# PRBonn/OverlapNet

Measured on AMD Instinct MI355X. Metric: scan-pairs/s (64x900 range images), higher is better.
Workload: dtype f32 (scaled 3-term fp16 split on the fp16 MFMA: 22 significand bits per operand, fp32 accumulate)

## Files before the change

overlapnet_amd/csrc/c3_dense.hip:

```cpp
#include "ovn_internal.h"

typedef _Float16 f16x8 __attribute__((ext_vector_type(8)));
typedef _Float16 f16x4 __attribute__((ext_vector_type(4)));

namespace {

struct ArithF16 {
  typedef _Float16 elem;
  typedef f16x8 v8;
  typedef f16x4 v4;
  static __device__ __forceinline__ f32x4 mfma(v8 a, v8 b, f32x4 c) { return __builtin_amdgcn_mfma_f32_16x16x32_f16(a, b, c, 0, 0, 0); }
};

constexpr int G = OVN_G;
constexpr int OW = OVN_O3_HW;
constexpr int CI = OVN_C2_OUT;
constexpr int CO = OVN_C3_OUT;
constexpr int NBAND = 3;
constexpr int MAX_ROWS = 8;
constexpr int MAX_MT = (MAX_ROWS * OW + 15) / 16;
constexpr int IN_PIX_MAX = (MAX_ROWS + 2) * G;
constexpr int PLANE = IN_PIX_MAX * 8 + 8;
constexpr int NPL = CI / 8;
constexpr size_t LDS_BYTES = 2 * (size_t)NPL * PLANE * sizeof(_Float16) + 64;
// ... 1 lines not shown

__device__ __forceinline__ int band_start(int b) { return b == 0 ? 0 : (b == 1 ? 8 : 15); }
__device__ __forceinline__ int band_rows(int b) { return b == 0 ? 8 : 7; }

constexpr int MT_SPLIT = 6;
template <class A, int NWV, int MSPLIT>
__global__ __launch_bounds__(64 * NWV) void c3_dense_kernel(const float* __restrict__ o2, const typename A::elem* __restrict__ wp,
                                                           const float* __restrict__ b3, const float* __restrict__ wd,
                                                           const unsigned* __restrict__ o2max, float sw3,
                                                           float* __restrict__ partial, float* __restrict__ o3,
                                                           unsigned* __restrict__ arrived, const float* __restrict__ bd,
                                                           float* __restrict__ overlap, float* __restrict__ logit) {
  typedef typename A::elem elem_t;
  typedef typename A::v8 v8_t;
  typedef typename A::v4 v4_t;
  extern __shared__ __attribute__((aligned(16))) unsigned char smem[];
  elem_t* ih = reinterpret_cast<elem_t*>(smem);
  elem_t* il = ih + NPL * PLANE;
  float* red = reinterpret_cast<float*>(il + NPL * PLANE);

  constexpr int HALVES = NW / NWV;
  constexpr int MTW = MSPLIT == 1 ? MAX_MT : MT_SPLIT;
  const int sub = blockIdx.x % (HALVES * MSPLIT);
  const int unit = blockIdx.x / (HALVES * MSPLIT), half = sub % HALVES, mh = sub / HALVES;
  const int mt0 = MT_SPLIT * mh;
  const int pair = unit / NBAND;
  const int band = unit - pair * NBAND;
  const int r0 = band_start(band);
  const int nrows = band_rows(band);
  const int npix = nrows * OW;
  const int nmt = (npix + 15) >> 4;
// ... 37 lines not shown
        const int c = 4 * (i - pix * (CI / 4));
        v4_t h, l;
#pragma unroll
        for (int e = 0; e < 4; ++e) {
          const float x = v[k][e] * s2;
          h[e] = (elem_t)x;
          l[e] = (elem_t)(x - (float)h[e]);
        }
        const int o = (c >> 3) * PLANE + pix * 8 + (c & 7);
        *reinterpret_cast<v4_t*>(ih + o) = h;
        *reinterpret_cast<v4_t*>(il + o) = l;
      }
    }
  }

  int abase[MTW];
#pragma unroll
  for (int mt = 0; mt < MTW; ++mt) {
    int p = 16 * (mt0 + mt) + lrow;
    if (p >= npix) p = npix - 1;
    const int oy = p / OW;
    const int ox = p - oy * OW;
    abase[mt] = g * PLANE + (oy * G + ox) * 8;
  }

  f32x4 acc[MTW][2];
#pragma unroll
  for (int mt = 0; mt < MTW; ++mt) {
    acc[mt][0] = (f32x4){0.f, 0.f, 0.f, 0.f};
    acc[mt][1] = (f32x4){0.f, 0.f, 0.f, 0.f};
  }

#define C3_MFMA2(M0, M1, A0H, A0L, A1H, A1L, SRC)                                                  \
  acc[M0][0] = A::mfma(A0H, SRC[0], acc[M0][0]);          \
  acc[M0][1] = A::mfma(A0H, SRC[2], acc[M0][1]);          \
  acc[M1][0] = A::mfma(A1H, SRC[0], acc[M1][0]);          \
  acc[M1][1] = A::mfma(A1H, SRC[2], acc[M1][1]);          \
  acc[M0][0] = A::mfma(A0L, SRC[0], acc[M0][0]);          \
  acc[M0][1] = A::mfma(A0L, SRC[2], acc[M0][1]);          \
  acc[M1][0] = A::mfma(A1L, SRC[0], acc[M1][0]);          \
  acc[M1][1] = A::mfma(A1L, SRC[2], acc[M1][1]);          \
  acc[M0][0] = A::mfma(A0H, SRC[1], acc[M0][0]);          \
  acc[M0][1] = A::mfma(A0H, SRC[3], acc[M0][1]);          \
  acc[M1][0] = A::mfma(A1H, SRC[1], acc[M1][0]);          \
  acc[M1][1] = A::mfma(A1H, SRC[3], acc[M1][1]);
#define C3_READ_A(BUF, SLOT, MT)                                                            \
  fh[BUF][SLOT] = *reinterpret_cast<const v8_t*>(ih + abase[MT] + toff);                  \
  fl[BUF][SLOT] = *reinterpret_cast<const v8_t*>(il + abase[MT] + toff);
#define C3_STEP(SRC, KC)                                                                    \
  {                                                                                         \
    const int tap = (KC) >> 2;                                                              \
    const int ky = tap / 3;                                                                 \
    const int toff = (ky * G + (tap - 3 * ky)) * 8 + 4 * PLANE * ((KC) & 3);                \
    v8_t fh[2][2], fl[2][2];                                                              \
    C3_READ_A(0, 0, 0)                                                                      \
    C3_READ_A(0, 1, 1)                                                                      \
    _Pragma("unroll") for (int q = 0; q < MTW / 2; ++q) {                                \
      const int cb = q & 1, nb = cb ^ 1;                                                    \
      if (q + 1 < MTW / 2) {                                                             \
        C3_READ_A(nb, 0, 2 * q + 2)                                                         \
        C3_READ_A(nb, 1, 2 * q + 3)                                                         \
      } else if (MTW % 2 == 1 && nmt == MAX_MT) {                                                           \
        C3_READ_A(nb, 0, MTW - 1)                                                        \
      }                                                                                     \
      __builtin_amdgcn_sched_barrier(0);   \
      C3_MFMA2(2 * q, 2 * q + 1, fh[cb][0], fl[cb][0], fh[cb][1], fl[cb][1], SRC)           \
      __builtin_amdgcn_sched_barrier(0);                                                    \
    }                                                                                       \
// ... 9 lines not shown
  }
  __syncthreads();
#pragma unroll 1
  for (int kc = 0; kc < 36; kc += 3) {
    C3_LOAD_B(bq[2], kc + 2)
    C3_STEP(bq[0], kc)
    if (kc + 3 < 36) C3_LOAD_B(bq[0], kc + 3)
    C3_STEP(bq[1], kc + 1)
    if (kc + 4 < 36) C3_LOAD_B(bq[1], kc + 4)
    C3_STEP(bq[2], kc + 2)
  }
#undef C3_LOAD_B
#undef C3_STEP
#undef C3_MFMA2
#undef C3_READ_A

  float s[2] = {0.f, 0.f};
#pragma unroll
  for (int nt = 0; nt < 2; ++nt) {
    const int n = 32 * wave + 16 * nt + lrow;
    const float bv = b3[n];
#pragma unroll
    for (int mt = 0; mt < MTW; ++mt) {
#pragma unroll
      for (int r = 0; r < 4; ++r) {
        const int p = 16 * (mt0 + mt) + 4 * g + r;
        if (p < npix) {
          const float v = fmaxf(fmaf(acc[mt][nt][r], inv, bv), 0.0f);
          const long long fi = (long long)(r0 * OW + p) * CO + n;
          s[(MSPLIT == 1 && mt >= MT_SPLIT) ? 1 : 0] += v * wd[fi];
// ... 58 lines not shown
  for (int b = 0; b < NBAND; ++b) {
    const float zb = (q[4 * b] + q[4 * b + 1]) + (q[4 * b + 2] + q[4 * b + 3]);
    z = b == 0 ? zb : z + zb;
  }
  z += bd[0];
  if (logit) logit[p] = z;
  overlap[p] = 1.0f / (1.0f + expf(-z));
}

}

int ovn_c3_dense_forward(const ovn_ctx* ctx, const float* o2, const unsigned* o2max, int n, float* partial, float* o3,
                         unsigned* arrived, float* overlap, float* logit, hipStream_t stream) {
  OVN_REQUIRE(o2max != nullptr, OVN_ERR_ARG, "ovn_c3_dense_forward: the per-pair maxima of o2 are required");
  OVN_REQUIRE(overlap == nullptr || arrived != nullptr, OVN_ERR_ARG, "ovn_c3_dense_forward: arrival counters missing");
  int rc;
  if (n <= 21) {
    rc = ovn_allow_dynamic_lds(reinterpret_cast<const void*>(c3_dense_kernel<ArithF16, 4, 2>), LDS_BYTES);
    if (rc) return rc;
    hipLaunchKernelGGL((c3_dense_kernel<ArithF16, 4, 2>), dim3(4 * NBAND * n), dim3(64 * 4), LDS_BYTES, stream, o2,
                       reinterpret_cast<const _Float16*>(ctx->c3.wp_h), ctx->c3.bias, ctx->wd, o2max, ctx->c3.sw_h, partial, o3, arrived,
                       ctx->bd, overlap, logit);
  } else {
    rc = ovn_allow_dynamic_lds(reinterpret_cast<const void*>(c3_dense_kernel<ArithF16, NW, 1>), LDS_BYTES);
    if (rc) return rc;
    hipLaunchKernelGGL((c3_dense_kernel<ArithF16, NW, 1>), dim3(NBAND * n), dim3(64 * NW), LDS_BYTES, stream, o2,
                       reinterpret_cast<const _Float16*>(ctx->c3.wp_h), ctx->c3.bias, ctx->wd, o2max, ctx->c3.sw_h, partial, o3,
                       (unsigned*)nullptr, ctx->bd, (float*)nullptr, (float*)nullptr);
    if (overlap != nullptr)
      hipLaunchKernelGGL(dense_finish_kernel, dim3((n + 255) / 256), dim3(256), 0, stream, partial, ctx->bd, n, overlap, logit);
  }
  OVN_HIP_CHECK(hipGetLastError());
  return OVN_OK;
}
```

overlapnet_amd/csrc/delta_head_f16x3.hip:

```cpp
#include <math.h>
#include <stdlib.h>

#include <type_traits>

#include "ovn_internal.h"
#include "delta_a2.h"

typedef _Float16 f16x8 __attribute__((ext_vector_type(8)));
typedef _Float16 f16x4 __attribute__((ext_vector_type(4)));
typedef _Float16 f16x2 __attribute__((ext_vector_type(2)));
typedef __bf16 bf16x8 __attribute__((ext_vector_type(8)));

namespace {

constexpr int FW = OVN_FEAT_W;
constexpr int FC = OVN_FEAT_C;
constexpr int S = OVN_S;
constexpr int G = OVN_G;
constexpr int O1 = OVN_C1_OUT;
constexpr int O2 = OVN_C2_OUT;
constexpr int K1 = S * FC;
constexpr int K2 = S * O1;
constexpr int STEP_BYTES = 8192;
constexpr int NWAVE = 8;
// ... 1331 lines not shown
    bool full = false;
    if constexpr (RT != 0) full = pass < NFULL;
    if constexpr (RT != 0) {
      if (full) run_pass(std::integral_constant<int, 0>{}, pass);
    }
    if (!full) {
      if (tail_slots == 2) run_pass(std::integral_constant<int, 2>{}, pass);
      else run_pass(std::integral_constant<int, 1>{}, pass);
    }
  }
#undef OVN_DMA_L
#undef OVN_DMA_W
#undef OVN_DMA_R
}

template <class AR, int MT, int ASLOTS, int WSETS>
__global__ __launch_bounds__(256, 2) void delta_c2_kernel(const float* __restrict__ o1raw, const void* __restrict__ w2p,
                                                          const DeltaDesc* __restrict__ desc, const f32x4* __restrict__ scales,
                                                          float* __restrict__ o2, unsigned* __restrict__ o2max, float one) {
  typedef typename AR::frag frag;
  constexpr int NPL = AR::PLANES;
  constexpr int SLAB = NPL * 8192;
  __shared__ __attribute__((aligned(16))) unsigned char wb[2][SLAB];
  constexpr int NKS = K2 / 32;
  constexpr int WG_ROWS = 64 * MT;
  static_assert(C2_TILE_ROWS % WG_ROWS == 0 && 6 % ASLOTS == 0 && 6 % WSETS == 0 && NKS % 6 == 0 && ASLOTS >= 2, "bad c_conv2 tiling");
  const int tid = threadIdx.x, lane = tid & 63;
  const int wave = __builtin_amdgcn_readfirstlane(tid >> 6);
  const int lrow = lane & 15, g = lane >> 4;
  const int wg_row0 = blockIdx.x * WG_ROWS;
  const int row0 = wg_row0 + 16 * MT * wave;
  const int tile = wg_row0 / C2_TILE_ROWS, in_tile = wg_row0 - tile * C2_TILE_ROWS;
  const float* abase = o1raw + (size_t)tile * (C2_TILE_ROWS * K2) + (in_tile + 16 * MT * wave + lrow) * 32 + 8 * g;
  const unsigned char* w2bytes = reinterpret_cast<const unsigned char*>(w2p) + tid * 16;

  f32x4 araw[ASLOTS][MT][2];
  f32x4 wr[WSETS][2 * NPL];
#define OVN_LOAD_A(SLOT, KS)                                                                 \
  _Pragma("unroll") for (int mt = 0; mt < MT; ++mt) {                                        \
    araw[SLOT][mt][0] = *reinterpret_cast<const f32x4*>(abase + (KS) * (C2_TILE_ROWS * 32) + mt * 512);       \
    araw[SLOT][mt][1] = *reinterpret_cast<const f32x4*>(abase + (KS) * (C2_TILE_ROWS * 32) + mt * 512 + 4);   \
  }
#define OVN_LOAD_W(SET, KS) \
  _Pragma("unroll") for (int q = 0; q < 2 * NPL; ++q) wr[SET][q] = *reinterpret_cast<const f32x4*>(w2bytes + (size_t)(KS) * SLAB + q * 4096);
#define OVN_STORE_W(SET, BUF) \
  _Pragma("unroll") for (int q = 0; q < 2 * NPL; ++q) *reinterpret_cast<f32x4*>(&wb[BUF][q * 4096 + tid * 16]) = wr[SET][q];

  f32x4 acc[MT][8];
#pragma unroll
  for (int mt = 0; mt < MT; ++mt)
#pragma unroll
    for (int nt = 0; nt < 8; ++nt) acc[mt][nt] = (f32x4){0.f, 0.f, 0.f, 0.f};

#pragma unroll
  for (int k = 0; k < WSETS; ++k) OVN_LOAD_W(k, k)
#pragma unroll
  for (int k = 0; k < ASLOTS - 1; ++k) OVN_LOAD_A(k, k)
  OVN_STORE_W(0, 0)
  __syncthreads();
// ... 4 lines not shown
    if ((KS) + WSETS < NKS) OVN_LOAD_W((J) % WSETS, (KS) + WSETS)                                                 \
    if ((KS) + ASLOTS - 1 < NKS) OVN_LOAD_A(((J) + ASLOTS - 1) % ASLOTS, (KS) + ASLOTS - 1)                       \
    __builtin_amdgcn_sched_barrier(0);         \
    frag af[MT][NPL];                                                                                             \
    _Pragma("unroll") for (int mt = 0; mt < MT; ++mt)                                                             \
      AR::split8(araw[(J) % ASLOTS][mt][0], araw[(J) % ASLOTS][mt][1], one, af[mt]);                              \
    const unsigned char* wcur = &wb[(J) & 1][lane * 16];                                                          \
    _Pragma("unroll") for (int nt = 0; nt < 8; ++nt) {                                                            \
      frag bf[NPL];                                                                                               \
      _Pragma("unroll") for (int pl = 0; pl < NPL; ++pl)                                                          \
        bf[pl] = *reinterpret_cast<const frag*>(wcur + (nt * NPL + pl) * 1024);                                   \
      _Pragma("unroll") for (int tm = 0; tm < AR::TERMS; ++tm)                                                    \
        _Pragma("unroll") for (int mt = 0; mt < MT; ++mt)                                                         \
          acc[mt][nt] = AR::mma(af[mt][AR::ta(tm)], bf[AR::tb(tm)], acc[mt][nt]);                                 \
    }                                                                                                             \
    if ((KS) + 1 < NKS) OVN_STORE_W(((J) + 1) % WSETS, ((J) + 1) & 1)                                             \
    __syncthreads();                                                                                              \
  }
#pragma unroll 1
  for (int ks = 0; ks < NKS; ks += 6) {
    OVN_C2_STEP(0, ks)
    OVN_C2_STEP(1, ks + 1)
    OVN_C2_STEP(2, ks + 2)
    OVN_C2_STEP(3, ks + 3)
    OVN_C2_STEP(4, ks + 4)
    OVN_C2_STEP(5, ks + 5)
  }
#undef OVN_C2_STEP
#undef OVN_LOAD_A
#undef OVN_LOAD_W
#undef OVN_STORE_W

  static_assert((G * G) % C2_TILE_ROWS == 0, "a c_conv2 workgroup must not straddle two pairs");
  const int pair = blockIdx.x / (G * G / WG_ROWS);
  const float inv2 = scales[2 * pair][3];
  typedef const __attribute__((address_space(1))) float* gfloat_p;
  const gfloat_p tt = (gfloat_p)desc[pair].tt;
  const gfloat_p aa = (gfloat_p)desc[pair].aa;
  float vmax = 0.f;
  float lv[2][8];
  auto load_lin = [&](int q, float* dst8) {
    const int rr = row0 + 16 * (q >> 2) - pair * (G * G) + 4 * g + (q & 3);
    const int jb = rr / G, ib = rr - jb * G;
#pragma unroll
    for (int nt = 0; nt < 8; ++nt) dst8[nt] = tt[ib * O2 + 16 * nt + lrow] + aa[jb * O2 + 16 * nt + lrow];
  };
  load_lin(0, lv[0]);
#pragma unroll
  for (int q = 0; q < 4 * MT; ++q) {
    if (q + 1 < 4 * MT) load_lin(q + 1, lv[(q + 1) & 1]);
    const int mt = q >> 2, r = q & 3;
    const int rr = row0 + 16 * mt - pair * (G * G) + 4 * g + r;
    const int jb = rr / G, ib = rr - jb * G;
    float* dst = o2 + (((size_t)pair * G + ib) * G + jb) * O2 + lrow;
#pragma unroll
    for (int nt = 0; nt < 8; ++nt) {
      const float v = fmaxf(fmaf(acc[mt][nt][r], inv2, lv[q & 1][nt]), 0.0f);
      dst[16 * nt] = v;
      vmax = fmaxf(vmax, v);
    }
  }
#pragma unroll
  for (int off = 32; off > 0; off >>= 1) vmax = fmaxf(vmax, __shfl_down(vmax, off, 64));
  if (lane == 0 && vmax > 0.f) atomicMax(o2max + pair, __float_as_uint(vmax));
}

}

size_t ovn_delta_f16x3_scratch_bytes(int n, bool per_pair_right) {
  auto al = [](size_t b) { return (b + 255) & ~(size_t)255; };
  return al((size_t)n * 8 * sizeof(float)) + al((size_t)n * sizeof(unsigned)) + 2 * al((size_t)n * OVN_FEAT_ELEMS * sizeof(unsigned)) +
         al((size_t)n * LIN_ELEMS * sizeof(float)) + al((size_t)(per_pair_right ? n : 1) * A2_KSPLIT * A2_ELEMS * sizeof(float)) +
         al((size_t)n * O1RAW_ELEMS * sizeof(float)) + al((size_t)n * sizeof(DeltaDesc)) + al(QBLOCK_WORDS * sizeof(unsigned)) +
         al(LIVE_WORDS * sizeof(unsigned)) + al((size_t)S * FC * O1 * 2 * sizeof(_Float16));
}

size_t ovn_delta_f16x3_seg_bytes(int nseg) {
  auto al = [](size_t b) { return (b + 255) & ~(size_t)255; };
  return al((size_t)nseg * A2_KSPLIT * A2_ELEMS * sizeof(float)) + al((size_t)nseg * QBLOCK_WORDS * sizeof(unsigned)) +
// ... 39 lines not shown
                     lidx, live, w1c, pseg, seg0);
  return OVN_OK;
}

template <class AR>
static int launch_c1(int n, int nsplit, const DeltaDesc* desc, const void* w1, const f32x4* scales, float* o1raw, int pair0,
                     const int32_t* lidx, const unsigned* live, const void* w1c, hipStream_t stream) {
  return launch_c1_t<AR, false>(n, nsplit, desc, w1, scales, o1raw, pair0, lidx, live, w1c, stream, nullptr, 0);
}

template <class AR>
static void launch_c2(int n, const float* o1raw, const void* w2, const DeltaDesc* desc, const f32x4* scales, float* o2, unsigned* o2max,
                      hipStream_t stream) {
  const int total_rows = n * G * G;
  if (n <= 28)
    hipLaunchKernelGGL((delta_c2_kernel<AR, 1, 6, 3>), dim3(total_rows / 64), dim3(256), 0, stream, o1raw, w2, desc, scales, o2, o2max, 1.0f);
  else
    hipLaunchKernelGGL((delta_c2_kernel<AR, 3, 3, 1>), dim3(total_rows / C2_TILE_ROWS), dim3(256), 0, stream, o1raw, w2, desc, scales, o2, o2max, 1.0f);
}

float* ovn_delta_f16x3_a2raw(void* scratch, int n) {
  auto al = [](size_t b) { return (b + 255) & ~(size_t)255; };
  char* p = static_cast<char*>(scratch);
  p += al((size_t)n * 8 * sizeof(float)) + al((size_t)n * sizeof(unsigned)) + 2 * al((size_t)n * OVN_FEAT_ELEMS * sizeof(unsigned)) +
       al((size_t)n * LIN_ELEMS * sizeof(float));
  return reinterpret_cast<float*>(p);
}

static int delta_c12_f16x3_segments(ovn_ctx* ctx, const float* feats_l, const int32_t* lidx, const float* feats_r, const int32_t* ridx,
                                    int n, void* scratch, unsigned** o2max_out, float* o2, hipStream_t stream, const float* dcache_l,
                                    const OvnSegPass& seg) {
  int rc = ovn_allow_dynamic_lds(reinterpret_cast<const void*>(delta_prepare_split_kernel<false, true>), PREP_SPLIT_LDS);
  if (rc) return rc;
// ... 37 lines not shown
  {
    OvnProfScope ps(ctx, OVN_K_DELTA, stream);
    rc = launch_c1_t<ArithF16x3, true>(n, nsplit, desc, ctx->w1p_h, scales, o1raw, 0, lidx, live, w1c, stream, seg.pseg, seg.seg0);
    if (rc) return rc;
  }
  {
    OvnProfScope ps(ctx, OVN_K_DELTA_C2, stream);
    launch_c2<ArithF16x3>(n, o1raw, ctx->w2p_h, desc, scales, o2, o2max, stream);
  }
  OVN_HIP_CHECK(hipGetLastError());
  return OVN_OK;
}

int ovn_delta_c12_f16x3_forward(ovn_ctx* ctx, const float* feats_l, const int32_t* lidx, const float* feats_r,
                                const int32_t* ridx, int n, void* scratch, unsigned** o2max_out, float* o2, hipStream_t stream,
                                int pair0, const float* dcache_l, bool a2_done, const OvnSegPass* seg) {
  int rc = ovn_allow_dynamic_lds(reinterpret_cast<const void*>(delta_prepare_split_kernel<false>), PREP_SPLIT_LDS);
  if (rc) return rc;
  if (seg) return delta_c12_f16x3_segments(ctx, feats_l, lidx, feats_r, ridx, n, scratch, o2max_out, o2, stream, dcache_l, *seg);
  if (ridx) dcache_l = nullptr;
  auto al = [](size_t b) { return (b + 255) & ~(size_t)255; };
  char* p = static_cast<char*>(scratch);
  f32x4* scales = reinterpret_cast<f32x4*>(p);
  p += al((size_t)n * 8 * sizeof(float));
  unsigned* o2max = reinterpret_cast<unsigned*>(p);
  p += al((size_t)n * sizeof(unsigned));
  unsigned* pl = reinterpret_cast<unsigned*>(p);
  p += al((size_t)n * OVN_FEAT_ELEMS * sizeof(unsigned));
  unsigned* pr = reinterpret_cast<unsigned*>(p);
  p += al((size_t)n * OVN_FEAT_ELEMS * sizeof(unsigned));
  float* lin = reinterpret_cast<float*>(p);
// ... 25 lines not shown
      hipLaunchKernelGGL(delta_live_kernel, dim3(1), dim3(512), 0, stream, feats_r, live_buf);
      hipLaunchKernelGGL(delta_w1c_kernel, dim3(240), dim3(256), 0, stream, reinterpret_cast<const _Float16*>(ctx->w1p_h), live, w1c);
    }
    hipLaunchKernelGGL(delta_prepare_split_kernel<false>, dim3(n), dim3(512), PREP_SPLIT_LDS, stream, feats_l, lidx, feats_r, ridx,
                       reinterpret_cast<const _Float16*>(ctx->wsp_h), ctx->w1col, ctx->b1, a2raw,
                       reinterpret_cast<const _Float16*>(ctx->w2p_h), ctx->w2sum, ctx->c2.bias, ctx->hs.sw1, ctx->hs.sw2, ctx->hs.sws,
                       ctx->hs.w1_colsum, ctx->hs.b1_absmax, 1.0f, scales, o2max, pl, pr, lin, desc, dcache_l, qblock, (float*)nullptr, live);
  }
  {
    OvnProfScope ps(ctx, OVN_K_DELTA, stream);
    rc = launch_c1<ArithF16x3>(n, nsplit, desc, ctx->w1p_h, scales, o1raw, pair0, lidx, live, w1c, stream);
    if (rc) return rc;
  }
  {
    OvnProfScope ps(ctx, OVN_K_DELTA_C2, stream);
    launch_c2<ArithF16x3>(n, o1raw, ctx->w2p_h, desc, scales, o2, o2max, stream);
  }
  OVN_HIP_CHECK(hipGetLastError());
  return OVN_OK;
}

int ovn_delta_c12_bf16x3_forward(ovn_ctx* ctx, const float* feats_l, const int32_t* lidx, const float* feats_r, const int32_t* ridx,
                                 int n, void* scratch, float* o2, hipStream_t stream, int pair0, bool a2_done) {
  int rc = ovn_allow_dynamic_lds(reinterpret_cast<const void*>(delta_prepare_bf16x3_kernel), PREP_B3_LDS);
  if (rc) return rc;
  auto al = [](size_t b) { return (b + 255) & ~(size_t)255; };
  char* p = static_cast<char*>(scratch);
  f32x4* scales = reinterpret_cast<f32x4*>(p);
  p += al((size_t)n * 8 * sizeof(float));
  unsigned* o2max = reinterpret_cast<unsigned*>(p);
  p += al((size_t)n * sizeof(unsigned));
  unsigned* pl = reinterpret_cast<unsigned*>(p);
// ... 124 lines not shown
```

overlapnet_amd/csrc/ovn_api.hip:

```cpp
#include <stdarg.h>
#include <mutex>
#include <set>
#include <utility>
#include <stdio.h>
#include <stdlib.h>
#include <string.h>

#include <algorithm>
#include "ovn_internal.h"

int ovn_allow_dynamic_lds(const void* kernel, size_t bytes) {
  static std::mutex mu;
  static std::set<std::pair<const void*, int>> done;
  int dev = 0;
  OVN_HIP_CHECK(hipGetDevice(&dev));
  std::lock_guard<std::mutex> lock(mu);
  if (done.count({kernel, dev})) return OVN_OK;
  OVN_HIP_CHECK(hipFuncSetAttribute(kernel, hipFuncAttributeMaxDynamicSharedMemorySize, (int)bytes));
  done.insert({kernel, dev});
  return OVN_OK;
}

static thread_local char g_err[1024] = "";

// ... 39 lines not shown
  OVN_REQUIRE(device_id >= 0 && device_id < ndev, OVN_ERR_ARG, "ovn_create: device %d not present (%d devices)", device_id, ndev);
  OVN_ON_DEVICE(device_id);
  hipDeviceProp_t prop;
  OVN_HIP_CHECK(hipGetDeviceProperties(&prop, device_id));
  OVN_REQUIRE(strncmp(prop.gcnArchName, "gfx950", 6) == 0, OVN_ERR_STATE,
              "ovn_create: this library is built for gfx950 only, device %d is %s", device_id, prop.gcnArchName);
  ovn_ctx* c = new ovn_ctx();
  c->device = device_id;
  c->in_h = in_h;
  c->in_w = in_w;
  c->in_c = in_c;
  if (const char* e = getenv("OVN_HEAD_CHUNK")) c->head_chunk = atoll(e) > 0 ? atoll(e) : c->head_chunk;
  if (const char* e = getenv("OVN_HEAD_SUBCHUNK")) c->head_sub = atoll(e) >= 0 ? atoll(e) : c->head_sub;
  if (const char* e = getenv("OVN_HEAD_STREAMS")) c->head_streams = atoi(e) == 2 ? 2 : 1;
  if (const char* e = getenv("OVN_YAW_SIDE")) c->head_yaw_side = atoi(e) ? 1 : 0;
  int rc = ovn_spectral_prepare(c, nullptr);
  if (rc) {
    ovn_conv_release(&c->dft);
    if (c->tw64) (void)hipFree(c->tw64);
    delete c;
    return rc;
  }
  *out = c;
  return OVN_OK;
}

int ovn_destroy(ovn_ctx* ctx) {
  if (!ctx) return OVN_OK;
  if (ctx->comm) (void)ovn_comm_destroy(ctx);
  OVN_ON_DEVICE(ctx->device);
// ... 20 lines not shown
  if (ctx->ws) (void)hipFree(ctx->ws);
  if (ctx->norm_buf) (void)hipFree(ctx->norm_buf);
  if (ctx->actmax) (void)hipFree(ctx->actmax);
  if (ctx->c3_arrived) (void)hipFree(ctx->c3_arrived);
  if (ctx->seg_dev) (void)hipFree(ctx->seg_dev);
  if (ctx->seg_host) (void)hipHostFree(ctx->seg_host);
  if (ctx->seg_ev) (void)hipEventDestroy(ctx->seg_ev);
  if (ctx->seg_done) (void)hipEventDestroy(ctx->seg_done);
  if (ctx->aux_ready) {
    for (int i = 0; i < 2; ++i) {
      (void)hipStreamDestroy(ctx->aux[i]);
      (void)hipEventDestroy(ctx->ev_join[i]);
    }
    (void)hipEventDestroy(ctx->ev_fork);
  }
  delete ctx;
  return OVN_OK;
}

int ovn_add_leg_layer(ovn_ctx* ctx, const char* name, const float* kernel_dev, const float* bias_dev, int kh, int kw,
                      int cin, int cout, int stride_h, int stride_w, void* stream) {
  OVN_REQUIRE(ctx && name && kernel_dev && bias_dev, OVN_ERR_ARG, "ovn_add_leg_layer: NULL argument");
  OVN_REQUIRE(kh > 0 && kw > 0 && cin > 0 && cout > 0 && stride_h > 0 && stride_w > 0, OVN_ERR_ARG,
              "ovn_add_leg_layer(%s): bad geometry", name);
  OVN_REQUIRE(!ctx->finalized, OVN_ERR_STATE, "ovn_add_leg_layer(%s): context already finalized", name);
  const int expect_cin = ctx->leg.empty() ? ctx->in_c : ctx->leg.back().cout;
  OVN_REQUIRE(cin == expect_cin, OVN_ERR_ARG, "ovn_add_leg_layer(%s): cin=%d but previous layer produces %d", name, cin, expect_cin);
  OVN_ON_DEVICE(ctx->device);
  OvnConvLayer L;
  L.name = name;
// ... 222 lines not shown
int ovn_corr_head_spectral(ovn_ctx* ctx, const float* spec_l, const int32_t* lidx, const float* spec_r,
                           const int32_t* ridx, int64_t n, int32_t* yaw, float* corr, void* stream) {
  OVN_REQUIRE(ctx != nullptr, OVN_ERR_ARG, "ovn_corr_head_spectral: ctx is NULL");
  OVN_REQUIRE(ctx_feat_w(ctx) == OVN_FEAT_W, OVN_ERR_ARG,
              "ovn_corr_head_spectral: the spectral correlation head needs 360-column feature volumes (the leg produces %d)", ctx_feat_w(ctx));
  OVN_REQUIRE(n >= 0 && n < (1ll << 31), OVN_ERR_ARG, "ovn_corr_head_spectral: bad n");
  if (n == 0) return OVN_OK;
  OVN_REQUIRE(spec_l && spec_r && yaw, OVN_ERR_ARG, "ovn_corr_head_spectral: NULL buffer");
  OVN_ON_DEVICE(ctx->device);
  OvnProfScope ps(ctx, OVN_K_CORR_SPECTRAL, (hipStream_t)stream);
  return ovn_corr_spectral_forward(ctx, spec_l, lidx, spec_r, ridx, (int)n, yaw, corr, (hipStream_t)stream);
}

static int head_streams_ready(ovn_ctx* ctx) {
  if (ctx->aux_ready) return OVN_OK;
  for (int i = 0; i < 2; ++i) {
    OVN_HIP_CHECK(hipStreamCreateWithFlags(&ctx->aux[i], hipStreamNonBlocking));
    OVN_HIP_CHECK(hipEventCreateWithFlags(&ctx->ev_join[i], hipEventDisableTiming));
  }
  OVN_HIP_CHECK(hipEventCreateWithFlags(&ctx->ev_fork, hipEventDisableTiming));
  ctx->aux_ready = true;
  return OVN_OK;
}

struct OvnFork {
  ovn_ctx* ctx;
  hipStream_t stream;
  bool used[2] = {false, false};
  bool forked = false;
  OvnFork(ovn_ctx* c, hipStream_t s) : ctx(c), stream(s) {}
  int fork() {
    if (forked) return OVN_OK;
// ... 70 lines not shown
    if (fusedc12) {
      rc = ovn_delta_forward(ctx, fl, li, feats_r, ri, np, ctx->ws, overlap + p0, logit ? logit + p0 : nullptr, stream);
    } else {
      OvnProfScope ps(ctx, OVN_K_DELTA, stream);
      rc = ovn_delta_generic_forward(ctx, fl, li, feats_r, ri, np, ctx->ws, overlap + p0, logit ? logit + p0 : nullptr, stream);
    }
    if (rc) return rc;
  }
  if (fusedc12 && n > 0 && n <= chunk) {
    const size_t o2w = (size_t)n * ctx->head_g * ctx->head_g * OVN_C2_OUT * sizeof(float);
    ctx->dbg_o2 = static_cast<const float*>(ctx->ws);
    ctx->dbg_o3 = reinterpret_cast<const float*>(static_cast<const char*>(ctx->ws) + ((o2w + 255) & ~(size_t)255));
    ctx->dbg_n = n;
  }
  return fk.join();
}

static int delta_head_run(ovn_ctx* ctx, const float* feats_l, const int32_t* lidx, const float* feats_r,
                          const int32_t* ridx, int64_t n, float* overlap, float* logit, int32_t* yaw, float* corr,
                          int corr_mode, const float* spec_l, const float* spec_r, const float* dcache_l, hipStream_t stream,
                          const OvnSegPass* seg = nullptr) {
  ctx->dbg_live = nullptr;
  const int fw = ctx_feat_w(ctx);
  if (ctx->head_s != OVN_S || fw != OVN_FEAT_W || ctx->head_mode == 0)
    return delta_head_run_f32(ctx, feats_l, lidx, feats_r, ridx, n, overlap, logit, yaw, corr, corr_mode, spec_l, spec_r, stream);
  const size_t feat_elems = (size_t)fw * OVN_FEAT_C;
  const size_t o2_elems = (size_t)OVN_G * OVN_G * OVN_C2_OUT;
  const size_t o3_elems = (size_t)OVN_DENSE_IN;
  const bool fused = (ctx->head_mode == 1);
  const int64_t chunk = ctx->head_chunk;
// ... 59 lines not shown
        if (rc) return rc;
      }
      const float* fl = lidx ? feats_l : feats_l + (size_t)p0 * feat_elems;
      const int32_t* li = lidx ? lidx + p0 : nullptr;
      const int32_t* ri = ridx ? ridx + p0 : nullptr;
      float* o2s = o2 + (size_t)q0 * o2_elems;
      if (fused) {
        unsigned* o2max = nullptr;
        float* part = o3 + (size_t)q0 * OVN_DENSE_PARTIALS;
        OvnSegPass sp{};
        if (seg) {
          sp = *seg;
          sp.pseg += p0;
          sp.scratch = dscratch + sc_sub * nsub_max;
        }
        rc = ovn_delta_c12_f16x3_forward(ctx, fl, li, feats_r, ri, np, dscratch + (size_t)j * sc_sub, &o2max, o2s, st, (int)(p0 & 0x3fffffff),
                                          dcache_l ? (lidx ? dcache_l : dcache_l + (size_t)p0 * OVN_DELTA_CACHE_ELEMS) : nullptr, a2_in_yaw,
                                          seg ? &sp : nullptr);
        if (rc) return rc;
        if (p0 == 0) ctx->dbg_o2max = o2max;
        {
          OvnProfScope ps(ctx, OVN_K_C3, st);
          rc = ovn_c3_dense_forward(ctx, o2s, o2max, np, part, nullptr, ctx->c3_arrived + q0, overlap + p0, logit ? logit + p0 : nullptr, st);
        }
      } else {
        float* o3s = o3 + (size_t)q0 * o3_elems;
        rc = ovn_delta_c12_bf16x3_forward(ctx, fl, li, feats_r, ri, np, dscratch + (size_t)j * sc_sub, o2s, st, (int)(p0 & 0x3fffffff),
                                          a2_in_yaw);
        if (rc) return rc;
        int oh = 0, ow = 0;
        {
          OvnProfScope ps(ctx, OVN_K_C3, st);
          rc = ovn_conv_forward(ctx->c3, o2s, np, OVN_G, OVN_G, o3s, &oh, &ow, st);
        }
        if (rc) return rc;
        OvnProfScope ps(ctx, OVN_K_DENSE, st);
// ... 466 lines not shown
```

overlapnet_amd/csrc/ovn_internal.h:

```cpp
#pragma once

#include <hip/hip_runtime.h>
#include <math.h>
#include <stdint.h>

#include <string>
#include <vector>

#include "../../include/ovn_hip.h"

typedef float f32x4 __attribute__((ext_vector_type(4)));

void ovn_set_error(const char* fmt, ...);

#define OVN_HIP_CHECK(expr)                                                                   \
  do {                                                                                        \
    hipError_t _e = (expr);                                                                   \
    if (_e != hipSuccess) {                                                                   \
      ovn_set_error("%s failed: %s (%s:%d)", #expr, hipGetErrorString(_e), __FILE__, __LINE__); \
      return OVN_ERR_HIP;                                                                     \
    }                                                                                         \
  } while (0)

#define OVN_REQUIRE(cond, code, ...)   \
// ... 213 lines not shown
  int head_mode = 1;
  int head_width_split = 0;
  float* wd = nullptr;
  float* bd = nullptr;
  OvnConvLayer dft;
  double* tw64 = nullptr;
  int corr_norm = 0;
  float* norm_buf = nullptr;
  int64_t norm_buf_n = 0;
  void* comm = nullptr;
  int comm_rank = 0, comm_world = 1;
  int64_t head_chunk = 1024;
  int64_t head_sub = 0;
  int head_streams = 1;
  int head_yaw_side = 0;
  bool aux_ready = false;
  hipStream_t aux[2] = {nullptr, nullptr};
  hipEvent_t ev_fork = nullptr, ev_join[2] = {nullptr, nullptr};
  void* ws = nullptr;
  size_t ws_bytes = 0;
  bool prof = false;
  struct ProfRec {
    hipEvent_t a, b;
    int kind;
  };
  std::vector<ProfRec> prof_recs;
  const float* dbg_o2 = nullptr;
  const float* dbg_o3 = nullptr;
  float* dbg_partial = nullptr;
  const unsigned* dbg_o2max = nullptr;
// ... 51 lines not shown
                            hipStream_t stream);
size_t ovn_delta_f16x3_scratch_bytes(int n, bool per_pair_right);
struct OvnSegPass {
  const int32_t* pseg;
  const int32_t* qidx;
  const int64_t* offs;
  int seg0, nseg;
  void* scratch;
};
size_t ovn_delta_f16x3_seg_bytes(int nseg);
int ovn_delta_c12_f16x3_forward(ovn_ctx* ctx, const float* feats_l, const int32_t* lidx, const float* feats_r,
                                const int32_t* ridx, int n, void* scratch, unsigned** o2max_out, float* o2, hipStream_t stream,
                                int pair0 = 0,
                                const float* dcache_l = nullptr,
                                bool a2_done = false,
                                const struct OvnSegPass* seg = nullptr);
float* ovn_delta_f16x3_a2raw(void* scratch, int n);
int ovn_delta_c12_bf16x3_forward(ovn_ctx* ctx, const float* feats_l, const int32_t* lidx, const float* feats_r, const int32_t* ridx,
                                 int n, void* scratch, float* o2, hipStream_t stream, int pair0, bool a2_done);
int ovn_delta_cache_forward(ovn_ctx* ctx, const float* feats, int n, float* cache, hipStream_t stream);
int ovn_delta_walk_stats(ovn_ctx* ctx, int32_t* out16, hipStream_t stream);

size_t ovn_delta_generic_pair_bytes(int W, int G);
int ovn_delta_generic_forward(const ovn_ctx* ctx, const float* feats_l, const int32_t* lidx, const float* feats_r,
                              const int32_t* ridx, int n, void* scratch, float* overlap, float* logit, hipStream_t stream);

size_t ovn_delta_w_split_pair_bytes();
int ovn_delta_w_split_c12_forward(ovn_ctx* ctx, const float* feats_l, const int32_t* lidx, const float* feats_r, const int32_t* ridx,
                                  int n, void* scales, float* o2, hipStream_t stream);

int ovn_corr_forward(const float* feats_l, const int32_t* lidx, const float* feats_r, const int32_t* ridx, int n, int W,
// ... 52 lines not shown
```

Baseline: 239,800.

## Add optional c2/c3 rider overlap, static LDS and cheaper c3 A-address math

```diff
diff --git a/overlapnet_amd/csrc/c3_dense.hip b/overlapnet_amd/csrc/c3_dense.hip
--- a/overlapnet_amd/csrc/c3_dense.hip
+++ b/overlapnet_amd/csrc/c3_dense.hip
@@ -39,7 +39,7 @@
   typedef typename A::elem elem_t;
   typedef typename A::v8 v8_t;
   typedef typename A::v4 v4_t;
-  extern __shared__ __attribute__((aligned(16))) unsigned char smem[];
+  __shared__ __attribute__((aligned(16))) unsigned char smem[LDS_BYTES];
   elem_t* ih = reinterpret_cast<elem_t*>(smem);
   elem_t* il = ih + NPL * PLANE;
   float* red = reinterpret_cast<float*>(il + NPL * PLANE);
@@ -107,14 +107,26 @@
     }
   }
 
-  int abase[MTW];
-#pragma unroll
-  for (int mt = 0; mt < MTW; ++mt) {
-    int p = 16 * (mt0 + mt) + lrow;
-    if (p >= npix) p = npix - 1;
-    const int oy = p / OW;
-    const int ox = p - oy * OW;
-    abase[mt] = g * PLANE + (oy * G + ox) * 8;
+  int abase[MSPLIT == 1 ? 1 : MTW];
+  int lbase = 0, a9 = 0;
+  unsigned rowbit = 0u;
+  if constexpr (MSPLIT == 1) {
+    lbase = g * PLANE + lrow * 8;
+#pragma unroll
+    for (int mt = 0; mt < MTW; ++mt) rowbit |= ((16 * mt) % OW + lrow >= OW ? 1u : 0u) << mt;
+    int p9 = 16 * 9 + lrow;
+    if (p9 >= npix) p9 = npix - 1;
+    a9 = g * PLANE + (p9 + 2 * (p9 / OW)) * 8;
+    abase[0] = 0;
+  } else {
+#pragma unroll
+    for (int mt = 0; mt < MTW; ++mt) {
+      int p = 16 * (mt0 + mt) + lrow;
+      if (p >= npix) p = npix - 1;
+      const int oy = p / OW;
+      const int ox = p - oy * OW;
+      abase[mt] = g * PLANE + (oy * G + ox) * 8;
+    }
   }
 
   f32x4 acc[MTW][2];
@@ -137,14 +149,20 @@
   acc[M0][1] = A::mfma(A0H, SRC[3], acc[M0][1]);          \
   acc[M1][0] = A::mfma(A1H, SRC[1], acc[M1][0]);          \
   acc[M1][1] = A::mfma(A1H, SRC[3], acc[M1][1]);
+#define C3_AOFF(MT)                                                                         \
+  (MSPLIT != 1 ? abase[MSPLIT != 1 ? (MT) : 0] + toff                                      \
+               : ((MT) == 9 ? a9 + toff : lt + (int)(((rb >> (MT)) & 1u) << 4) + (128 * (MT) + 16 * ((16 * (MT)) / OW))))
 #define C3_READ_A(BUF, SLOT, MT)                                                            \
-  fh[BUF][SLOT] = *reinterpret_cast<const v8_t*>(ih + abase[MT] + toff);                  \
-  fl[BUF][SLOT] = *reinterpret_cast<const v8_t*>(il + abase[MT] + toff);
+  fh[BUF][SLOT] = *reinterpret_cast<const v8_t*>(ih + C3_AOFF(MT));                       \
+  fl[BUF][SLOT] = *reinterpret_cast<const v8_t*>(il + C3_AOFF(MT));
 #define C3_STEP(SRC, KC)                                                                    \
   {                                                                                         \
     const int tap = (KC) >> 2;                                                              \
     const int ky = tap / 3;                                                                 \
     const int toff = (ky * G + (tap - 3 * ky)) * 8 + 4 * PLANE * ((KC) & 3);                \
+    const int lt = lbase + toff;                                                            \
+    unsigned rb = rowbit;                                                                   \
+    asm volatile("" : "+v"(rb));    \
     v8_t fh[2][2], fl[2][2];                                                              \
     C3_READ_A(0, 0, 0)                                                                      \
     C3_READ_A(0, 1, 1)                                                                      \
@@ -184,6 +202,7 @@
 #undef C3_STEP
 #undef C3_MFMA2
 #undef C3_READ_A
+#undef C3_AOFF
 
   float s[2] = {0.f, 0.f};
 #pragma unroll
@@ -272,17 +291,12 @@
                          unsigned* arrived, float* overlap, float* logit, hipStream_t stream) {
   OVN_REQUIRE(o2max != nullptr, OVN_ERR_ARG, "ovn_c3_dense_forward: the per-pair maxima of o2 are required");
   OVN_REQUIRE(overlap == nullptr || arrived != nullptr, OVN_ERR_ARG, "ovn_c3_dense_forward: arrival counters missing");
-  int rc;
   if (n <= 21) {
-    rc = ovn_allow_dynamic_lds(reinterpret_cast<const void*>(c3_dense_kernel<ArithF16, 4, 2>), LDS_BYTES);
-    if (rc) return rc;
-    hipLaunchKernelGGL((c3_dense_kernel<ArithF16, 4, 2>), dim3(4 * NBAND * n), dim3(64 * 4), LDS_BYTES, stream, o2,
+    hipLaunchKernelGGL((c3_dense_kernel<ArithF16, 4, 2>), dim3(4 * NBAND * n), dim3(64 * 4), 0, stream, o2,
                        reinterpret_cast<const _Float16*>(ctx->c3.wp_h), ctx->c3.bias, ctx->wd, o2max, ctx->c3.sw_h, partial, o3, arrived,
                        ctx->bd, overlap, logit);
   } else {
-    rc = ovn_allow_dynamic_lds(reinterpret_cast<const void*>(c3_dense_kernel<ArithF16, NW, 1>), LDS_BYTES);
-    if (rc) return rc;
-    hipLaunchKernelGGL((c3_dense_kernel<ArithF16, NW, 1>), dim3(NBAND * n), dim3(64 * NW), LDS_BYTES, stream, o2,
+    hipLaunchKernelGGL((c3_dense_kernel<ArithF16, NW, 1>), dim3(NBAND * n), dim3(64 * NW), 0, stream, o2,
                        reinterpret_cast<const _Float16*>(ctx->c3.wp_h), ctx->c3.bias, ctx->wd, o2max, ctx->c3.sw_h, partial, o3,
                        (unsigned*)nullptr, ctx->bd, (float*)nullptr, (float*)nullptr);
     if (overlap != nullptr)
diff --git a/overlapnet_amd/csrc/delta_head_f16x3.hip b/overlapnet_amd/csrc/delta_head_f16x3.hip
--- a/overlapnet_amd/csrc/delta_head_f16x3.hip
+++ b/overlapnet_amd/csrc/delta_head_f16x3.hip
@@ -1369,10 +1369,11 @@
 #undef OVN_DMA_R
 }
 
-template <class AR, int MT, int ASLOTS, int WSETS>
-__global__ __launch_bounds__(256, 2) void delta_c2_kernel(const float* __restrict__ o1raw, const void* __restrict__ w2p,
-                                                          const DeltaDesc* __restrict__ desc, const f32x4* __restrict__ scales,
-                                                          float* __restrict__ o2, unsigned* __restrict__ o2max, float one) {
+template <class AR, int MT, int ASLOTS, int WSETS, bool WALK = false>
+__global__ __launch_bounds__(256, WALK ? 4 : 2) void delta_c2_kernel(const float* __restrict__ o1raw, const void* __restrict__ w2p,
+                                                                     const DeltaDesc* __restrict__ desc, const f32x4* __restrict__ scales,
+                                                                     float* __restrict__ o2, unsigned* __restrict__ o2max, float one,
+                                                                     int nwg) {
   typedef typename AR::frag frag;
   constexpr int NPL = AR::PLANES;
   constexpr int SLAB = NPL * 8192;
@@ -1380,24 +1381,30 @@
   constexpr int NKS = K2 / 32;
   constexpr int WG_ROWS = 64 * MT;
   static_assert(C2_TILE_ROWS % WG_ROWS == 0 && 6 % ASLOTS == 0 && 6 % WSETS == 0 && NKS % 6 == 0 && ASLOTS >= 2, "bad c_conv2 tiling");
-  const int tid = threadIdx.x, lane = tid & 63;
-  const int wave = __builtin_amdgcn_readfirstlane(tid >> 6);
+  const int wave = __builtin_amdgcn_readfirstlane((int)threadIdx.x >> 6);
+  int wg = blockIdx.x;
+  do {
+  int lane = (int)threadIdx.x & 63;
+  if constexpr (WALK) asm volatile("v_mbcnt_lo_u32_b32 %0, -1, 0\n\tv_mbcnt_hi_u32_b32 %0, -1, %0" : "=v"(lane));
+  const int tid = 64 * wave + lane;
   const int lrow = lane & 15, g = lane >> 4;
-  const int wg_row0 = blockIdx.x * WG_ROWS;
+  const int wg_row0 = wg * WG_ROWS;
   const int row0 = wg_row0 + 16 * MT * wave;
   const int tile = wg_row0 / C2_TILE_ROWS, in_tile = wg_row0 - tile * C2_TILE_ROWS;
-  const float* abase = o1raw + (size_t)tile * (C2_TILE_ROWS * K2) + (in_tile + 16 * MT * wave + lrow) * 32 + 8 * g;
-  const unsigned char* w2bytes = reinterpret_cast<const unsigned char*>(w2p) + tid * 16;
+  const float* abase = o1raw + (size_t)tile * (C2_TILE_ROWS * K2) + (in_tile + 16 * MT * wave) * 32;
+  const unsigned aoff = (unsigned)(lrow * 32 + 8 * g);
+  const unsigned char* w2bytes = reinterpret_cast<const unsigned char*>(w2p);
+  const unsigned woff = (unsigned)tid * 16u;
 
   f32x4 araw[ASLOTS][MT][2];
   f32x4 wr[WSETS][2 * NPL];
 #define OVN_LOAD_A(SLOT, KS)                                                                 \
   _Pragma("unroll") for (int mt = 0; mt < MT; ++mt) {                                        \
-    araw[SLOT][mt][0] = *reinterpret_cast<const f32x4*>(abase + (KS) * (C2_TILE_ROWS * 32) + mt * 512);       \
-    araw[SLOT][mt][1] = *reinterpret_cast<const f32x4*>(abase + (KS) * (C2_TILE_ROWS * 32) + mt * 512 + 4);   \
+    araw[SLOT][mt][0] = *reinterpret_cast<const f32x4*>(abase + (KS) * (C2_TILE_ROWS * 32) + mt * 512 + aoff);       \
+    araw[SLOT][mt][1] = *reinterpret_cast<const f32x4*>(abase + (KS) * (C2_TILE_ROWS * 32) + mt * 512 + 4 + aoff);   \
   }
 #define OVN_LOAD_W(SET, KS) \
-  _Pragma("unroll") for (int q = 0; q < 2 * NPL; ++q) wr[SET][q] = *reinterpret_cast<const f32x4*>(w2bytes + (size_t)(KS) * SLAB + q * 4096);
+  _Pragma("unroll") for (int q = 0; q < 2 * NPL; ++q) wr[SET][q] = *reinterpret_cast<const f32x4*>(w2bytes + (size_t)(KS) * SLAB + q * 4096 + woff);
 #define OVN_STORE_W(SET, BUF) \
   _Pragma("unroll") for (int q = 0; q < 2 * NPL; ++q) *reinterpret_cast<f32x4*>(&wb[BUF][q * 4096 + tid * 16]) = wr[SET][q];
 
@@ -1432,6 +1439,9 @@
         _Pragma("unroll") for (int mt = 0; mt < MT; ++mt)                                                         \
           acc[mt][nt] = AR::mma(af[mt][AR::ta(tm)], bf[AR::tb(tm)], acc[mt][nt]);                                 \
     }                                                                                                             \
+     \
+     \
+    __builtin_amdgcn_sched_barrier(0);                                                                            \
     if ((KS) + 1 < NKS) OVN_STORE_W(((J) + 1) % WSETS, ((J) + 1) & 1)                                             \
     __syncthreads();                                                                                              \
   }
@@ -1450,7 +1460,7 @@
 #undef OVN_STORE_W
 
   static_assert((G * G) % C2_TILE_ROWS == 0, "a c_conv2 workgroup must not straddle two pairs");
-  const int pair = blockIdx.x / (G * G / WG_ROWS);
+  const int pair = wg / (G * G / WG_ROWS);
   const float inv2 = scales[2 * pair][3];
   typedef const __attribute__((address_space(1))) float* gfloat_p;
   const gfloat_p tt = (gfloat_p)desc[pair].tt;
@@ -1481,6 +1491,9 @@
 #pragma unroll
   for (int off = 32; off > 0; off >>= 1) vmax = fmaxf(vmax, __shfl_down(vmax, off, 64));
   if (lane == 0 && vmax > 0.f) atomicMax(o2max + pair, __float_as_uint(vmax));
+  if constexpr (!WALK) break;
+  wg += gridDim.x;
+  } while (wg < nwg);
 }
 
 }
@@ -1550,9 +1563,16 @@
                       hipStream_t stream) {
   const int total_rows = n * G * G;
   if (n <= 28)
-    hipLaunchKernelGGL((delta_c2_kernel<AR, 1, 6, 3>), dim3(total_rows / 64), dim3(256), 0, stream, o1raw, w2, desc, scales, o2, o2max, 1.0f);
+    hipLaunchKernelGGL((delta_c2_kernel<AR, 1, 6, 3>), dim3(total_rows / 64), dim3(256), 0, stream, o1raw, w2, desc, scales, o2, o2max, 1.0f, 0);
   else
-    hipLaunchKernelGGL((delta_c2_kernel<AR, 3, 3, 1>), dim3(total_rows / C2_TILE_ROWS), dim3(256), 0, stream, o1raw, w2, desc, scales, o2, o2max, 1.0f);
+    hipLaunchKernelGGL((delta_c2_kernel<AR, 3, 3, 1>), dim3(total_rows / C2_TILE_ROWS), dim3(256), 0, stream, o1raw, w2, desc, scales, o2, o2max, 1.0f, 0);
+}
+
+static void launch_c2_rider(int n, int grid, const float* o1raw, const void* w2, const DeltaDesc* desc, const f32x4* scales, float* o2,
+                            unsigned* o2max, hipStream_t stream) {
+  const int nwg = n * (G * G / 64);
+  hipLaunchKernelGGL((delta_c2_kernel<ArithF16x3, 1, 6, 1, true>), dim3(grid > 0 && grid < nwg ? grid : nwg), dim3(256), 0, stream, o1raw, w2,
+                     desc, scales, o2, o2max, 1.0f, nwg);
 }
 
 float* ovn_delta_f16x3_a2raw(void* scratch, int n) {
@@ -1620,7 +1640,7 @@
 
 int ovn_delta_c12_f16x3_forward(ovn_ctx* ctx, const float* feats_l, const int32_t* lidx, const float* feats_r,
                                 const int32_t* ridx, int n, void* scratch, unsigned** o2max_out, float* o2, hipStream_t stream,
-                                int pair0, const float* dcache_l, bool a2_done, const OvnSegPass* seg) {
+                                int pair0, const float* dcache_l, bool a2_done, const OvnSegPass* seg, int c2_pairs) {
   int rc = ovn_allow_dynamic_lds(reinterpret_cast<const void*>(delta_prepare_split_kernel<false>), PREP_SPLIT_LDS);
   if (rc) return rc;
   if (seg) return delta_c12_f16x3_segments(ctx, feats_l, lidx, feats_r, ridx, n, scratch, o2max_out, o2, stream, dcache_l, *seg);
@@ -1676,8 +1696,27 @@
   }
   {
     OvnProfScope ps(ctx, OVN_K_DELTA_C2, stream);
-    launch_c2<ArithF16x3>(n, o1raw, ctx->w2p_h, desc, scales, o2, o2max, stream);
-  }
+    launch_c2<ArithF16x3>(c2_pairs >= 0 && c2_pairs < n ? c2_pairs : n, o1raw, ctx->w2p_h, desc, scales, o2, o2max, stream);
+  }
+  OVN_HIP_CHECK(hipGetLastError());
+  return OVN_OK;
+}
+
+int ovn_delta_c2_f16x3_block(ovn_ctx* ctx, void* scratch, int n, bool per_pair_right, int p0, int np, float* o2, int grid,
+                             hipStream_t stream) {
+  auto al = [](size_t b) { return (b + 255) & ~(size_t)255; };
+  char* p = static_cast<char*>(scratch);
+  const f32x4* scales = reinterpret_cast<const f32x4*>(p);
+  p += al((size_t)n * 8 * sizeof(float));
+  unsigned* o2max = reinterpret_cast<unsigned*>(p);
+  p += al((size_t)n * sizeof(unsigned)) + 2 * al((size_t)n * OVN_FEAT_ELEMS * sizeof(unsigned)) + al((size_t)n * LIN_ELEMS * sizeof(float)) +
+       al((size_t)(per_pair_right ? n : 1) * A2_KSPLIT * A2_ELEMS * sizeof(float));
+  const float* o1raw = reinterpret_cast<const float*>(p);
+  p += al((size_t)n * O1RAW_ELEMS * sizeof(float));
+  const DeltaDesc* desc = reinterpret_cast<const DeltaDesc*>(p);
+  OvnProfScope ps(ctx, OVN_K_DELTA_C2, stream);
+  launch_c2_rider(np, grid, o1raw + (size_t)p0 * O1RAW_ELEMS, ctx->w2p_h, desc + p0, scales + 2 * (size_t)p0,
+                  o2 + (size_t)p0 * G * G * O2, o2max + p0, stream);
   OVN_HIP_CHECK(hipGetLastError());
   return OVN_OK;
 }
diff --git a/overlapnet_amd/csrc/ovn_api.hip b/overlapnet_amd/csrc/ovn_api.hip
--- a/overlapnet_amd/csrc/ovn_api.hip
+++ b/overlapnet_amd/csrc/ovn_api.hip
@@ -77,6 +77,10 @@
   if (const char* e = getenv("OVN_HEAD_SUBCHUNK")) c->head_sub = atoll(e) >= 0 ? atoll(e) : c->head_sub;
   if (const char* e = getenv("OVN_HEAD_STREAMS")) c->head_streams = atoi(e) == 2 ? 2 : 1;
   if (const char* e = getenv("OVN_YAW_SIDE")) c->head_yaw_side = atoi(e) ? 1 : 0;
+  if (const char* e = getenv("OVN_HEAD_RIDER")) c->head_rider = atoi(e) ? 1 : 0;
+  if (const char* e = getenv("OVN_HEAD_RIDER_BLOCK")) c->head_rider_block = atoll(e) > 0 ? atoll(e) : c->head_rider_block;
+  if (const char* e = getenv("OVN_HEAD_RIDER_GRID")) c->head_rider_grid = atoi(e) > 0 ? atoi(e) : 0;
+  if (const char* e = getenv("OVN_HEAD_RIDER_PRIO")) c->head_rider_prio = atoi(e) ? 1 : 0;
   int rc = ovn_spectral_prepare(c, nullptr);
   if (rc) {
     ovn_conv_release(&c->dft);
@@ -127,6 +131,7 @@
     }
     (void)hipEventDestroy(ctx->ev_fork);
   }
+  for (hipEvent_t e : ctx->ev_ride) (void)hipEventDestroy(e);
   delete ctx;
   return OVN_OK;
 }
@@ -379,8 +384,10 @@
 
 static int head_streams_ready(ovn_ctx* ctx) {
   if (ctx->aux_ready) return OVN_OK;
+  int prio_low = 0, prio_high = 0;
+  OVN_HIP_CHECK(hipDeviceGetStreamPriorityRange(&prio_low, &prio_high));
   for (int i = 0; i < 2; ++i) {
-    OVN_HIP_CHECK(hipStreamCreateWithFlags(&ctx->aux[i], hipStreamNonBlocking));
+    OVN_HIP_CHECK(hipStreamCreateWithPriority(&ctx->aux[i], hipStreamNonBlocking, (i == 0 && ctx->head_rider_prio) ? prio_low : 0));
     OVN_HIP_CHECK(hipEventCreateWithFlags(&ctx->ev_join[i], hipEventDisableTiming));
   }
   OVN_HIP_CHECK(hipEventCreateWithFlags(&ctx->ev_fork, hipEventDisableTiming));
@@ -481,6 +488,39 @@
     ctx->dbg_n = n;
   }
   return fk.join();
+}
+
+static int delta_head_ride(ovn_ctx* ctx, OvnFork& fk, void* dscratch, bool per_pair_right, int np, int block, float* o2s,
+                           const unsigned* o2max, float* part, unsigned* arrived, float* overlap, float* logit, hipStream_t st) {
+  hipStream_t rs = nullptr;
+  int rc = fk.side(0, &rs);
+  if (rc) return rc;
+  const int nb = (np + block - 1) / block;
+  while ((int)ctx->ev_ride.size() < nb) {
+    hipEvent_t e = nullptr;
+    OVN_HIP_CHECK(hipEventCreateWithFlags(&e, hipEventDisableTiming));
+    ctx->ev_ride.push_back(e);
+  }
+  OVN_HIP_CHECK(hipEventRecord(ctx->ev_ride[0], st));
+  OVN_HIP_CHECK(hipStreamWaitEvent(rs, ctx->ev_ride[0], 0));
+  const size_t o2_elems = (size_t)OVN_G * OVN_G * OVN_C2_OUT;
+  for (int k = 0; k < nb; ++k) {
+    const int b0 = k * block, bn = (np - b0 < block) ? np - b0 : block;
+    if (k > 0) OVN_HIP_CHECK(hipStreamWaitEvent(st, ctx->ev_ride[k], 0));
+    {
+      OvnProfScope ps(ctx, OVN_K_C3, st);
+      rc = ovn_c3_dense_forward(ctx, o2s + (size_t)b0 * o2_elems, o2max + b0, bn, part + (size_t)b0 * OVN_DENSE_PARTIALS, nullptr, arrived + b0,
+                                overlap + b0, logit ? logit + b0 : nullptr, st);
+    }
+    if (rc) return rc;
+    if (k + 1 < nb) {
+      const int r0 = b0 + block, rn = (np - r0 < block) ? np - r0 : block;
+      rc = ovn_delta_c2_f16x3_block(ctx, dscratch, np, per_pair_right, r0, rn, o2s, ctx->head_rider_grid, rs);
+      if (rc) return rc;
+      OVN_HIP_CHECK(hipEventRecord(ctx->ev_ride[k + 1], rs));
+    }
+  }
+  return OVN_OK;
 }
 
 static int delta_head_run(ovn_ctx* ctx, const float* feats_l, const int32_t* lidx, const float* feats_r,
@@ -570,12 +610,17 @@
           sp.pseg += p0;
           sp.scratch = dscratch + sc_sub * nsub_max;
         }
+        const int64_t rblock = ctx->head_rider_block;
+        const bool ride = ctx->head_rider && !seg && ctx->head_streams == 1 && nsub_max == 1 && np >= 2 * rblock;
         rc = ovn_delta_c12_f16x3_forward(ctx, fl, li, feats_r, ri, np, dscratch + (size_t)j * sc_sub, &o2max, o2s, st, (int)(p0 & 0x3fffffff),
                                           dcache_l ? (lidx ? dcache_l : dcache_l + (size_t)p0 * OVN_DELTA_CACHE_ELEMS) : nullptr, a2_in_yaw,
-                                          seg ? &sp : nullptr);
+                                          seg ? &sp : nullptr, ride ? (int)rblock : -1);
         if (rc) return rc;
         if (p0 == 0) ctx->dbg_o2max = o2max;
-        {
+        if (ride) {
+          rc = delta_head_ride(ctx, fk, dscratch + (size_t)j * sc_sub, ri != nullptr, np, (int)rblock, o2s, o2max, part, ctx->c3_arrived + q0,
+                               overlap + p0, logit ? logit + p0 : nullptr, st);
+        } else {
           OvnProfScope ps(ctx, OVN_K_C3, st);
           rc = ovn_c3_dense_forward(ctx, o2s, o2max, np, part, nullptr, ctx->c3_arrived + q0, overlap + p0, logit ? logit + p0 : nullptr, st);
         }
diff --git a/overlapnet_amd/csrc/ovn_internal.h b/overlapnet_amd/csrc/ovn_internal.h
--- a/overlapnet_amd/csrc/ovn_internal.h
+++ b/overlapnet_amd/csrc/ovn_internal.h
@@ -251,6 +251,11 @@
   int64_t head_sub = 0;
   int head_streams = 1;
   int head_yaw_side = 0;
+  int head_rider = 0;
+  int64_t head_rider_block = 256;
+  int head_rider_grid = 0;
+  int head_rider_prio = 0;
+  std::vector<hipEvent_t> ev_ride;
   bool aux_ready = false;
   hipStream_t aux[2] = {nullptr, nullptr};
   hipEvent_t ev_fork = nullptr, ev_join[2] = {nullptr, nullptr};
@@ -332,7 +337,10 @@
                                 int pair0 = 0,
                                 const float* dcache_l = nullptr,
                                 bool a2_done = false,
-                                const struct OvnSegPass* seg = nullptr);
+                                const struct OvnSegPass* seg = nullptr,
+                                int c2_pairs = -1);
+int ovn_delta_c2_f16x3_block(ovn_ctx* ctx, void* scratch, int n, bool per_pair_right, int p0, int np, float* o2, int grid,
+                             hipStream_t stream);
 float* ovn_delta_f16x3_a2raw(void* scratch, int n);
 int ovn_delta_c12_bf16x3_forward(ovn_ctx* ctx, const float* feats_l, const int32_t* lidx, const float* feats_r, const int32_t* ridx,
                                  int n, void* scratch, float* o2, hipStream_t stream, int pair0, bool a2_done);
```

Result: no change. 242,000, median of 6 (+0.9%).
